# bderembl/msom

Measured on NVIDIA B200. Metric: cell-layer updates/s, higher is better.
Workload: dtype f64

## Files before the change

msom_b200/csrc/model.cu:

```cuda
#include "../../include/msqg.h"
#include "layout.cuh"
#include "mg_kernels.cuh"
#include "rb_kernels.cuh"
#include "rhs_kernels.cuh"

#include <cmath>
#include <cstdio>
#include <cstdlib>
#include <cstring>
#include <dlfcn.h>
#include <vector>
#include <utility>
#include <map>
#include <tuple>
#include <thread>
#include <mutex>
#include <condition_variable>
#include <string>
#include <atomic>

static thread_local char g_err[512] = "";
static std::mutex g_kernel_init_mu;
extern "C" const char *msqg_last_error(void) { return g_err; }
#define FAIL(code, ...)                        \
// ... 977 lines not shown
    else {
      cudaLaunchConfig_t cfg;
      memset(&cfg, 0, sizeof(cfg));
      cudaLaunchAttribute at[1];
      at[0].id = cudaLaunchAttributeClusterDimension;
      at[0].val.clusterDim.x = cs; at[0].val.clusterDim.y = 1; at[0].val.clusterDim.z = 1;
      cfg.gridDim = dim3(cs * m->num_sms); cfg.blockDim = dim3(64 * WPC); cfg.dynamicSmemBytes = smem; cfg.attrs = at; cfg.numAttrs = 1;
      int ncl = 0;
      if (cudaOccupancyMaxActiveClusters(&ncl, (void *)kern, &cfg) != cudaSuccess || ncl < 1) {
        cudaGetLastError();
        m->relax_cs_ok = false;
        if (init_lk.owns_lock()) init_lk.unlock();
        return launch_relax_ws_w<NL, K, WPC, RCOEF>(m, da, res, lev, nsweeps, C);
      }
      max_blocks[tv] = ncl * cs;
    }
    attr_set[tv].store(true, std::memory_order_release);
  }
  if (init_lk.owns_lock()) init_lk.unlock();
  const int grid = (nworkers + WPC - 1) / WPC;
  int cap = cs == 1 ? max_blocks[tv] * m->num_sms : max_blocks[tv];
  { const char *e = getenv("MSQG_RELAX_CAP"); if (e && atoi(e) > 0 && atoi(e) < cap) cap = atoi(e); }
  if (cs > 1) cap = cap < cs ? cs : cap - cap % cs;
  if (cap < 1) FAIL(MSQG_ERR_ARG, "relax kernel does not fit on the device (nl=%d)", NL);
  RelaxCoef<NL> Cc = C;
  for (int b0 = 0; b0 < grid; b0 += cap) {
    A.w_base = b0 * WPC;
    const int nb = grid - b0 < cap ? grid - b0 : cap;
    void *args[] = {(void *)&A, (void *)&Cc};
    if (cs == 1) CK(cudaLaunchCooperativeKernel((void *)kern, dim3(nb), dim3(64 * WPC), args, smem, m->stream));
    else {
      cudaLaunchConfig_t cfg;
      memset(&cfg, 0, sizeof(cfg));
      cudaLaunchAttribute at[2];
      at[0].id = cudaLaunchAttributeClusterDimension;
      at[0].val.clusterDim.x = cs; at[0].val.clusterDim.y = 1; at[0].val.clusterDim.z = 1;
      at[1].id = cudaLaunchAttributeCooperative; at[1].val.cooperative = 1;
      cfg.gridDim = dim3((nb + cs - 1) / cs * cs); cfg.blockDim = dim3(64 * WPC); cfg.dynamicSmemBytes = smem; cfg.stream = m->stream;
      cfg.attrs = at; cfg.numAttrs = 2;
      CK(cudaLaunchKernelExC(&cfg, (void *)kern, args));
    }
    m->launches++;
  }
  return MSQG_OK;
}
template <int NL>
static int launch_relax_rowcoef(msqg_model *m, double *da, const double *res, int lev, int nsweeps, const RelaxCoef<NL> &C) {
  if constexpr (NL <= 6) {
    constexpr size_t spw = WsCfg<NL, 4>::smem_per_worker;
    if constexpr (spw * 4 <= 220 * 1024) return launch_relax_ws_w<NL, 4, 4, true>(m, da, res, lev, nsweeps, C);
    else return launch_relax_ws_w<NL, 4, 2, true>(m, da, res, lev, nsweeps, C);
  } else {
    FAIL(MSQG_ERR_ARG, "varRo > 0 with the layer-coupled solver is built for nl <= 6 (nl = %d)", NL);
  }
}
template <int NL, int K>
static int launch_relax_ws(msqg_model *m, double *da, const double *res, int lev, int nsweeps, const RelaxCoef<NL> &C) {
  constexpr size_t spw = WsCfg<NL, K>::smem_per_worker;
  if constexpr (spw * 4 <= 220 * 1024) return launch_relax_ws_w<NL, K, 4>(m, da, res, lev, nsweeps, C);
  else if constexpr (spw * 2 <= 220 * 1024) return launch_relax_ws_w<NL, K, 2>(m, da, res, lev, nsweeps, C);
  else return launch_relax_ws_w<NL, K, 1>(m, da, res, lev, nsweeps, C);
}
static int relax_variant() {
#ifdef MSQG_EXPERIMENTS
  static int v = -1;
  if (v < 0) { const char *e = getenv("MSQG_RELAX"); v = (e && !strcmp(e, "v3")) ? 0 : 1; }
  return v;
#else
  return 1;
#endif
}

#ifdef MSQG_EXPERIMENTS
template <int NL, int K>
static int launch_relax_w_t(msqg_model *m, double *da, const double *res, int lev, int nsweeps, const RelaxCoef<NL> &C) {
  constexpr size_t spw = RelaxCfg<NL, K>::smem_per_warp;
  if constexpr (spw * 4 <= 200 * 1024) return launch_relax_w<NL, K, 4>(m, da, res, lev, nsweeps, C);
  else return launch_relax_w<NL, K, 2>(m, da, res, lev, nsweeps, C);
}
#endif

template <int NL>
static int launch_relax_rb(msqg_model *m, double *da, const double *res, int lev, int nrelax, const RelaxCoef<NL> &C,
                           const int *orange, int halo);
template <int NL>
static int launch_relax(msqg_model *m, double *da, const double *res, int lev, int nrelax, const RelaxCoef<NL> &C) {
  if (m->smoother == 1) return launch_relax_rb<NL>(m, da, res, lev, nrelax, C, nullptr, 0);
  int done = 0;
  while (done < nrelax) {
    int ns = nrelax - done;
    int rc;
    if (relax_uses_table<NL>(m)) { if (ns > 4) ns = 4; rc = launch_relax_rowcoef<NL>(m, da, res, lev, ns, C); }
    else if (relax_variant() == 1) { if (ns > 4) ns = 4; rc = launch_relax_ws<NL, 4>(m, da, res, lev, ns, C); }
#ifdef MSQG_EXPERIMENTS
    else if (ns <= 4) rc = launch_relax_w_t<NL, 4>(m, da, res, lev, ns, C);
    else { if (ns > 8) ns = 8; rc = launch_relax_w_t<NL, 8>(m, da, res, lev, ns, C); }
#else
    else rc = MSQG_ERR_ARG;
#endif
    if (rc) return rc;
    done += ns;
  }
  return MSQG_OK;
}


struct KernelDevState { std::atomic<bool> set[64]; int occ[64][RB_NSMAX + 1]; };
template <int NL, bool RCOEF, int WXT>
static int launch_relax_rb_pass_w(msqg_model *m, double *da, const double *res, int lev, int ns, const RelaxCoef<NL> &C,
                                const int *orange , int halo) {
  using Cfg = RbCfg<NL, WXT>;
  const Geom &g = m->g[lev];
  const int nh = 2 * ns;
  if (da != m->da.lev[lev]) FAIL(MSQG_ERR_ARG, "the rb relax pass works on the model's da list");
  if (!m->da2.lev[lev]) {
    int rc = alloc_level(m, m->da2, m->nl, lev);
    if (rc) return rc;
    m->da2.nf = m->nl;
  }
  RbArgs A;
  memset(&A, 0, sizeof(A));
  A.da = da; A.da_out = m->da2.lev[lev]; A.res = res; A.g = g; A.ns = ns;
  A.R = 2 * nh + 1 + RB_PF;
  A.TX = WXT - 2 * nh;
  A.ox_lo = 0; A.ox_hi = g.nx; A.oy_lo = 0; A.oy_hi = g.ny;
  if (orange) { A.ox_lo = orange[0]; A.ox_hi = orange[1]; A.oy_lo = orange[2]; A.oy_hi = orange[3]; }
  A.xlo = (g.bc & 1) ? -halo : 0; A.xhi = g.nx + ((g.bc & 2) ? halo : 0);
  A.ylo = (g.bc & 4) ? -halo : 0; A.yhi = g.ny + ((g.bc & 8) ? halo : 0);
  A.par0 = 0;
  A.coef = RCOEF ? relax_table(m, lev) : nullptr;
  A.coef_cell = (RCOEF && relax_table_per_cell(m)) ? 1 : 0;
  A.reuse = m->rb_reuse;
  if (RCOEF && (g.bc || !A.coef)) FAIL(MSQG_ERR_ARG, "horizontally varying stretching (varRo, frpg) is supported on undecomposed levels only");
  const int nxo_ = A.ox_hi - A.ox_lo, nyo_ = A.oy_hi - A.oy_lo;
  if constexpr (NL <= 4) {
    int lim = 512;
    { const char *e = getenv("MSQG_RB_TILE"); if (e) lim = atoi(e); }
    if (RCOEF) { const char *e = getenv("MSQG_RB_COARSE_TABLES"); if (e && atoi(e) == 0) lim = 0; }
    if ((long long)nxo_ * nyo_ <= (long long)lim * lim) {
      constexpr int WS = RB_TO + 4 * RB_NSMAX;
      const size_t tsmem = (size_t)2 * NL * WS * WS * sizeof(double);
      auto tk = k_relax_rb_tile<NL, RCOEF>;
      static KernelDevState tst;
      const int dev = m->device & 63;
      if (!tst.set[dev].load(std::memory_order_acquire)) {
        std::lock_guard<std::mutex> lk(g_kernel_init_mu);
        if (!tst.set[dev].load(std::memory_order_relaxed)) {
          CK(cudaFuncSetAttribute(tk, cudaFuncAttributeMaxDynamicSharedMemorySize, (int)tsmem));
          tst.set[dev].store(true, std::memory_order_release);
        }
      }
      RelaxCoef<NL> Cc = C;
      tk<<<dim3((nxo_ + RB_TO - 1) / RB_TO, (nyo_ + RB_TO - 1) / RB_TO), 512, tsmem, m->stream>>>(A, Cc);
      m->launches++;
      CK(cudaGetLastError());
      std::swap(m->da.lev[lev], m->da2.lev[lev]);
      if (m->swap_log) m->swap_log->push_back({m->tile_index, lev});
      return MSQG_OK;
    }
  }
  const size_t smem = (size_t)A.R * Cfg::row_bytes;
  const int threads = Cfg::NSMAX * WXT;
  auto kern = k_relax_rb<NL, RCOEF, WXT>;
  static KernelDevState st;
  const int dev = m->device & 63;
  if (!st.set[dev].load(std::memory_order_acquire)) {
    std::lock_guard<std::mutex> lk(g_kernel_init_mu);
    if (!st.set[dev].load(std::memory_order_relaxed)) {
      CK(cudaFuncSetAttribute(kern, cudaFuncAttributeMaxDynamicSharedMemorySize,
                              (int)((size_t)(4 * Cfg::NSMAX + 1 + RB_PF) * Cfg::row_bytes)));
      for (int s = 1; s <= Cfg::NSMAX; s++)
        CK(cudaOccupancyMaxActiveBlocksPerMultiprocessor(&st.occ[dev][s], kern, Cfg::NSMAX * WXT,
                                                         (size_t)(4 * s + 1 + RB_PF) * Cfg::row_bytes));
      st.set[dev].store(true, std::memory_order_release);
    }
  }
  const int occ = st.occ[dev][ns] > 0 ? st.occ[dev][ns] : 1;
  const int nxo = A.ox_hi - A.ox_lo, nyo = A.oy_hi - A.oy_lo;
  const int nstrips = (nxo + A.TX - 1) / A.TX;
  int nchunks = (m->num_sms * occ) / nstrips;
  if (nchunks > nyo / 32) nchunks = nyo / 32;
  if (nchunks < 1) nchunks = 1;
  A.rpc = (nyo + nchunks - 1) / nchunks;
  nchunks = (nyo + A.rpc - 1) / A.rpc;
  RelaxCoef<NL> Cc = C;
  kern<<<dim3(nstrips, nchunks), threads, smem, m->stream>>>(A, Cc);
  m->launches++;
  CK(cudaGetLastError());
  std::swap(m->da.lev[lev], m->da2.lev[lev]);
  if (m->swap_log) m->swap_log->push_back({m->tile_index, lev});
  return MSQG_OK;
}
template <int NL, bool RCOEF>
static int launch_relax_rb_pass(msqg_model *m, double *da, const double *res, int lev, int ns, const RelaxCoef<NL> &C,
                                const int *orange, int halo) {
#ifdef MSQG_EXPERIMENTS
  int wx = 128;
  { const char *e = getenv("MSQG_RB_WX"); if (e) wx = atoi(e); }
  if constexpr (NL <= 4) {
    const Geom &g = m->g[lev];
    const long long cells = (long long)(orange ? orange[1] - orange[0] : g.nx) * (orange ? orange[3] - orange[2] : g.ny);
    long long minside = 1024;
    { const char *e = getenv("MSQG_RB_WX_MIN"); if (e) minside = atoi(e); }
    if (wx == 64 && cells >= minside * minside) return launch_relax_rb_pass_w<NL, RCOEF, 64>(m, da, res, lev, ns, C, orange, halo);
  }
#endif
  return launch_relax_rb_pass_w<NL, RCOEF, RB_WX>(m, da, res, lev, ns, C, orange, halo);
}
template <int NL>
static int launch_relax_rb(msqg_model *m, double *da, const double *res, int lev, int nrelax, const RelaxCoef<NL> &C,
                           const int *orange = nullptr, int halo = 0) {
  constexpr int NSMAX = RbCfg<NL>::NSMAX;
  int left = nrelax;
  if (da != m->da.lev[lev]) FAIL(MSQG_ERR_ARG, "the rb relax pass works on the model's da list");
  if (orange && nrelax > NSMAX) FAIL(MSQG_ERR_ARG, "a tile relax pass holds at most %d sweeps", NSMAX);
  while (left > 0) {
    const int passes = (left + NSMAX - 1) / NSMAX;
    const int ns = (left + passes - 1) / passes;
    int rc;
    if (relax_uses_table<NL>(m)) {
      if constexpr (NL <= 6) rc = launch_relax_rb_pass<NL, true>(m, m->da.lev[lev], res, lev, ns, C, orange, halo);
      else FAIL(MSQG_ERR_ARG, "varRo > 0 with the layer-coupled solver is built for nl <= 6 (nl = %d)", NL);
    } else
      rc = launch_relax_rb_pass<NL, false>(m, m->da.lev[lev], res, lev, ns, C, orange, halo);
    if (rc) return rc;
    left -= ns;
  }
  return MSQG_OK;
}

static int coarse_top_level(msqg_model *m, int nf_problem, int maxlevel) {
  if (m->smoother != 1) return 0;
  if (nf_problem > 1 && !m->s_uniform && (m->nl > 6 || !m->rowcoef[1] || m->g[1].bc)) return 0;
  if (nf_problem == 1 && !m->modes_uniform && !m->modecoef[0][1]) return 0;
  { const char *e = getenv("MSQG_RB_COARSE_TABLES");
    if (e && atoi(e) == 0 && (nf_problem > 1 ? !m->s_uniform : !m->modes_uniform)) return 0; }
  if (!m->periodic) { const char *e = getenv("MSQG_RB_COARSE"); if (e && atoi(e) == 0) return 0; }
  int Lc = coarse_max_level(nf_problem);
  if (Lc > maxlevel) Lc = maxlevel;
  return Lc >= 2 ? Lc : 0;
}
template <int NL, bool RCOEF = false>
static int launch_coarse_rb(msqg_model *m, int Lc, int nrelax, const CoarseCoef<NL> &CC) {
  CoarseArgs A;
  memset(&A, 0, sizeof(A));
  A.res = m->res.lev[Lc]; A.da = m->da.lev[Lc]; A.g = m->g[Lc]; A.Lc = Lc; A.nrelax = nrelax; A.periodic = m->periodic;
  if (RCOEF) {
    for (int l = 1; l <= Lc; l++) {
      A.coef[l] = relax_table(m, l);
      if (!A.coef[l]) FAIL(MSQG_ERR_ARG, "no coefficient table on level %d", l);
    }
    A.coef_cell = relax_table_per_cell(m) ? 1 : 0;
  }
  size_t cells = 0;
  for (int l = 1; l <= Lc; l++) cells += (size_t)1 << (2 * l);
  const size_t smem = 2 * (size_t)NL * cells * sizeof(double);
  auto kern = k_coarse_rb<NL, RCOEF>;
  static KernelDevState st;
  const int dev = m->device & 63;
  if (!st.set[dev].load(std::memory_order_acquire)) {
    std::lock_guard<std::mutex> lk(g_kernel_init_mu);
    if (!st.set[dev].load(std::memory_order_relaxed)) {
      CK(cudaFuncSetAttribute(kern, cudaFuncAttributeMaxDynamicSharedMemorySize, RB_COARSE_SMEM));
      st.set[dev].store(true, std::memory_order_release);
    }
  }
  CoarseCoef<NL> Cc = CC;
  kern<<<1, 512, smem, m->stream>>>(A, Cc);
  m->launches++;
  CK(cudaGetLastError());
  return MSQG_OK;
}

#define NL_CASE(n, ...) case n: { constexpr int NL = n; __VA_ARGS__; } break;
#define NL_SWITCH(nl, ...)                                  \
  switch (nl) {                                             \
    NL_CASE(2, __VA_ARGS__) NL_CASE(3, __VA_ARGS__) NL_CASE(4, __VA_ARGS__) NL_CASE(5, __VA_ARGS__)   \
    NL_CASE(6, __VA_ARGS__) NL_CASE(7, __VA_ARGS__) NL_CASE(8, __VA_ARGS__) NL_CASE(9, __VA_ARGS__)   \
    NL_CASE(10, __VA_ARGS__) NL_CASE(11, __VA_ARGS__) NL_CASE(12, __VA_ARGS__)                        \
    default: FAIL(MSQG_ERR_ARG, "unsupported nl=%d", nl);   \
  }

template <class T>
__global__ void k_to_host(T *__restrict__ dst_mapped, const T *__restrict__ src, int n) {
  const int i = threadIdx.x;
  if (i < n) dst_mapped[i] = src[i];
  __threadfence_system();
}
template <class T>
static inline cudaError_t to_host(cudaStream_t st, T *host_mapped, const T *dev, int n) {
  k_to_host<T><<<1, 64, 0, st>>>(host_mapped, dev, n);
  return cudaGetLastError();
}

__global__ void k_zero_words(double *p, int n) { if ((int)threadIdx.x < n) p[threadIdx.x] = 0.; }
static inline cudaError_t zero_words(cudaStream_t st, double *p, int n) {
  k_zero_words<<<1, 64, 0, st>>>(p, n);
  return cudaGetLastError();
}

static int check_relax_err(msqg_model *m) {
  CK(to_host(m->stream, m->h_err, m->d_err, 1));
  CK(cudaStreamSynchronize(m->stream));
  if (*m->h_err) {
    CK(cudaMemsetAsync(m->d_err, 0, sizeof(int), m->stream));
    k_fill_u64<<<m->num_sms * 4, 256, 0, m->stream>>>(m->mailbox, m->mailbox_words, MAIL_EMPTY);
    FAIL(MSQG_ERR_CUDA, "relax wavefront timed out waiting on a neighbour strip");
// ... 32 lines not shown
  if (rc) return rc;
  CK(cudaStreamSynchronize(m->stream));
  *maxres = m->h_scal[0];
  return MSQG_OK;
}

template <class F>
static int run_graphed(cudaStream_t st, GraphCache &gc, const GraphKey &key, std::vector<msqg_model *> &models, long *exchanges, bool enabled,
                       F body) {
  if (!enabled) return body();
  auto it = gc.entries.find(key);
  if (it != gc.entries.end()) {
    GraphEntry &E = it->second;
    CK(cudaGraphLaunch(E.exec, st));
    for (auto &sw : E.swaps) { msqg_model *m = models[sw.first]; std::swap(m->da.lev[sw.second], m->da2.lev[sw.second]); }
    models[0]->launches += E.launches;
    if (exchanges) *exchanges += E.exchanges;
    return MSQG_OK;
  }
  if (gc.seen[key]++ == 0) return body();
  GraphEntry E;
  long l0 = 0, x0 = exchanges ? *exchanges : 0;
  for (msqg_model *m : models) { l0 += m->launches; m->swap_log = &E.swaps; }
  cudaError_t e = cudaStreamBeginCapture(st, cudaStreamCaptureModeRelaxed);
  int rc = e == cudaSuccess ? body() : MSQG_ERR_CUDA;
  cudaGraph_t g = nullptr;
  cudaError_t e2 = cudaStreamEndCapture(st, &g);
  long l1 = 0;
  for (msqg_model *m : models) { l1 += m->launches; m->swap_log = nullptr; }
  if (e != cudaSuccess || rc || e2 != cudaSuccess || !g) {
    if (g) cudaGraphDestroy(g);
    cudaGetLastError();
    if (rc) return rc;
    FAIL(MSQG_ERR_CUDA, "recording the multigrid cycle as a CUDA graph failed: %s", cudaGetErrorString(e != cudaSuccess ? e : e2));
  }
  e = cudaGraphInstantiate(&E.exec, g, 0);
  cudaGraphDestroy(g);
  if (e != cudaSuccess) FAIL(MSQG_ERR_CUDA, "cudaGraphInstantiate: %s", cudaGetErrorString(e));
  E.launches = l1 - l0; E.exchanges = exchanges ? *exchanges - x0 : 0;
  CK(cudaGraphLaunch(E.exec, st));
  gc.entries[key] = E;
  return MSQG_OK;
}
static unsigned long long da_parity_mask(msqg_model *m) {
  unsigned long long mask = 0;
  for (int l = 1; l <= m->depth; l++)
    if (m->da.lev[l] && m->da.base[l] && m->da.lev[l] != m->da.base[l] + (size_t)(m->fy[l] - 1) * m->g[l].pitch) mask |= 1ull << l;
  return mask;
}

static int mg_fused(msqg_model *m, const MgProblem &P) {
#ifdef MSQG_EXPERIMENTS
  static int v = -1;
  if (v < 0) { const char *e = getenv("MSQG_MG"); v = (e && !strcmp(e, "rr")) ? 1 : (e && !strcmp(e, "fused")) ? 2 : 0; }
  const Geom &g = m->g[m->depth];
  return (P.mode < 0 && g.bc == 0 && m->depth >= 1 && !(g.nx & 1) && !(g.ny & 1) && m->smoother == 0) ? v : 0;
#else
  (void)m; (void)P;
  return 0;
#endif
}
#ifdef MSQG_EXPERIMENTS
static int mg_corr_residual(msqg_model *m, const MgProblem &P, const double *da, double *a_new, double *maxres) {
  const int D = m->depth;
  const Geom &g = m->g[D];
  CK(zero_words(m->stream, m->d_scal, 1));
  dim3 b(CR_BX, CR_BY);
  double *res_c = (D - 1 >= 1) ? m->res.lev[D - 1] : nullptr;
  const Geom &gc = m->g[D >= 1 ? D - 1 : 0];
  { ProfScope ps(m, PROF_RESIDUAL, 0);
    LayerMetrics M = metrics_of(m);
    if (da) { NL_SWITCH(m->nl, k_corr_res<NL, true><<<grid2(g.nx, g.ny, b), b, 0, m->stream>>>(P.a, da, a_new, P.b, m->res.lev[D], res_c, m->str.lev[D], g, gc, M, m->d_scal)); }
    else { NL_SWITCH(m->nl, k_corr_res<NL, false><<<grid2(g.nx, g.ny, b), b, 0, m->stream>>>(P.a, nullptr, nullptr, P.b, m->res.lev[D], res_c, m->str.lev[D], g, gc, M, m->d_scal)); }
  }
  m->launches++;
  CK(cudaGetLastError());
  CK(to_host(m->stream, m->h_scal, m->d_scal, 1));
  CK(cudaStreamSynchronize(m->stream));
  *maxres = m->h_scal[0];
  return MSQG_OK;
}

#endif
static int mg_levels(msqg_model *m, int nf, int mode, int nrelax, int from, int top) {
  dim3 b(32, 8);
  const int D = m->depth;
  const int Lc = coarse_top_level(m, nf, top < D ? top : D - 1);
  if (m->periodic && Lc < top) FAIL(MSQG_ERR_ARG, "periodic level %d is not covered by the wrap-around coarse kernel (levels 1 .. %d)", top, Lc);
  for (int l = from - 1; l >= (Lc ? Lc : 1); l--) {
    ProfScope ps(m, PROF_RESTRICT, l);
    k_restrict<<<grid2(m->g[l].nx, m->g[l].ny, b, nf), b, 0, m->stream>>>(m->res.lev[l + 1], m->res.lev[l], m->g[l + 1], m->g[l], -1., 0);
    m->launches++;
  }
  CK(cudaGetLastError());
  int rc = MSQG_OK;
  if (Lc) {
    ProfScope ps(m, PROF_RELAX_COARSE, nrelax);
    if (mode < 0) {
      NL_SWITCH(m->nl, {
        CoarseCoef<NL> CC;
        for (int l = 1; l <= Lc; l++) CC.c[l] = relax_coef_layers<NL>(m, l);
        CC.c[0] = CC.c[1];
        if (relax_uses_table<NL>(m)) {
          if constexpr (NL <= 6) rc = launch_coarse_rb<NL, true>(m, Lc, nrelax, CC);
          else rc = MSQG_ERR_ARG;
        } else
          rc = launch_coarse_rb<NL>(m, Lc, nrelax, CC);
      });
    } else {
      CoarseCoef<1> CC;
      for (int l = 1; l <= Lc; l++) CC.c[l] = relax_coef_scalar(m, l, m->lam_lev[(size_t)l * m->nl + mode]);
      CC.c[0] = CC.c[1];
      m->coef_mode = m->modes_uniform ? -1 : mode;
      rc = m->coef_mode >= 0 ? launch_coarse_rb<1, true>(m, Lc, nrelax, CC) : launch_coarse_rb<1>(m, Lc, nrelax, CC);
      m->coef_mode = -1;
    }
    if (rc) return rc;
  }
  const int minlevel = top < 1 ? top : 1;
  for (int l = Lc ? Lc + 1 : minlevel; l <= top; l++) {
    const Geom &g = m->g[l];
    if (l == minlevel) {
      CK(cudaMemsetAsync(m->da.lev[l], 0, (size_t)nf * g.plane * sizeof(double), m->stream));
    } else {
      ProfScope ps(m, PROF_PROLONG, l);
      launch_prolong(m->stream, nf, m->da.lev[l - 1], m->da.lev[l], m->g[l - 1], g);
      m->launches++;
      CK(cudaGetLastError());
    }
    ProfScope ps(m, l == D ? PROF_RELAX_FINE : PROF_RELAX_COARSE, nrelax);
    if (mode < 0) {
      NL_SWITCH(m->nl, { auto C = relax_coef_layers<NL>(m, l); rc = launch_relax<NL>(m, m->da.lev[l], m->res.lev[l], l, nrelax, C); });
    } else {
      auto C = relax_coef_scalar(m, l, m->lam_lev[(size_t)l * m->nl + mode]);
      m->coef_mode = m->modes_uniform ? -1 : mode;
      rc = launch_relax<1>(m, m->da.lev[l], m->res.lev[l], l, nrelax, C);
      m->coef_mode = -1;
    }
    if (rc) return rc;
  }
  return MSQG_OK;
}

static int mg_cycle(msqg_model *m, const MgProblem &P, int nrelax, int fused = 0) {
  const int D = m->depth;
  dim3 b(32, 8);
  int rc = mg_levels(m, P.nf, P.mode, nrelax, fused ? D - 1 : D, D);
  if (rc) return rc;
  if (fused == 2) return MSQG_OK;
  const Geom &g = m->g[D];
  { ProfScope ps(m, PROF_CORRECT, 0);
  k_correct<<<grid2(g.nx, g.ny, b, P.nf), b, 0, m->stream>>>(P.a, m->da.lev[D], g); }
  m->launches++;
  CK(cudaGetLastError());
  return MSQG_OK;
}

static int mg_solve(msqg_model *m, const MgProblem &P, double tolerance, msqg_mgstats *st) {
  msqg_mgstats s;
  memset(&s, 0, sizeof(s));
  s.nrelax = 4;
  double resb;
  int rc;
  const int fmode = mg_fused(m, P);
#ifdef MSQG_EXPERIMENTS
  if (fmode == 1) {
    if ((rc = mg_corr_residual(m, P, nullptr, nullptr, &resb))) return rc;
    s.resb = s.resa = resb;
    for (s.i = 0; s.i < 100 && (s.i < 1 || s.resa > tolerance); s.i++) {
      if ((rc = mg_cycle(m, P, s.nrelax, 1))) return rc;
      if ((rc = mg_corr_residual(m, P, nullptr, nullptr, &s.resa))) return rc;
      if (s.resa > tolerance) {
        if (resb / s.resa < 1.2 && s.nrelax < 100) s.nrelax++;
        else if (resb / s.resa > 10 && s.nrelax > 2) s.nrelax--;
      }
      resb = s.resa;
    }
  } else if (fmode == 2) {
    const int D = m->depth;
    if (!m->a_alt.lev[D] || m->a_alt.nf < P.nf) {
      free_list(m->a_alt);
      if ((rc = alloc_list(m, m->a_alt, P.nf, -1., D, D))) return rc;
    }
    MgProblem Q = P;
    double *other = m->a_alt.lev[D];
    if ((rc = mg_corr_residual(m, Q, nullptr, nullptr, &resb))) return rc;
    s.resb = s.resa = resb;
    for (s.i = 0; s.i < 100 && (s.i < 1 || s.resa > tolerance); s.i++) {
      if ((rc = mg_cycle(m, Q, s.nrelax, 2))) return rc;
      if ((rc = mg_corr_residual(m, Q, m->da.lev[D], other, &s.resa))) return rc;
      std::swap(Q.a, other);
      if (s.resa > tolerance) {
        if (resb / s.resa < 1.2 && s.nrelax < 100) s.nrelax++;
        else if (resb / s.resa > 10 && s.nrelax > 2) s.nrelax--;
      }
      resb = s.resa;
    }
    if (Q.a != P.a) {
      if (P.owner && *P.owner == P.a) { *P.owner = Q.a; m->a_alt.lev[D] = P.a; }
      else CK(cudaMemcpyAsync(P.a, Q.a, (size_t)P.nf * m->g[D].plane * sizeof(double), cudaMemcpyDeviceToDevice, m->stream));
    }
  } else
#else
  (void)fmode;
#endif
  {
  rc = mg_residual(m, P, &resb);
  if (rc) return rc;
  s.resb = s.resa = resb;
  const bool graphed = m->smoother == 1 && m->use_graphs && !m->prof_on;
  std::vector<msqg_model *> self(1, m);
  for (s.i = 0; s.i < 100 && (s.i < 1 || s.resa > tolerance); s.i++) {
    GraphKey key(s.nrelax, P.mode, (const void *)P.a, (const void *)P.b, da_parity_mask(m));
    rc = run_graphed(m->stream, m->graphs, key, self, nullptr, graphed, [&]() -> int {
      int r2 = mg_cycle(m, P, s.nrelax);
      if (r2) return r2;
      return mg_residual_enqueue(m, P);
    });
    if (rc) return rc;
    CK(cudaStreamSynchronize(m->stream));
    s.resa = m->h_scal[0];
    if (s.resa > tolerance) {
      if (resb / s.resa < 1.2 && s.nrelax < 100) s.nrelax++;
      else if (resb / s.resa > 10 && s.nrelax > 2) s.nrelax--;
    }
    resb = s.resa;
  }
  }
  if ((rc = check_relax_err(m))) return rc;
  m->total_cycles += s.i;
  *st = s;
  return MSQG_OK;
// ... 1078 lines not shown
```

msom_b200/csrc/rb_kernels.cuh:

```cuda
#pragma once
#include "mg_kernels.cuh"

#define RB_WX 128
#define RB_NP 64
#define RB_PF 4
#define RB_NSMAX 4

struct RbArgs {
  const double *da;
  double *da_out;
  const double *res;
  Geom g;
  int ns;
  int R;
  int TX;
  int rpc;
  int ox_lo, ox_hi, oy_lo, oy_hi;
  int xlo, xhi, ylo, yhi;
  int par0;
  const double *coef;
  int coef_cell;
  int reuse;
};

__device__ __forceinline__ void cp_async8(unsigned smem_addr, const void *gsrc) {
  asm volatile("cp.async.ca.shared.global [%0], [%1], 8;\n" ::"r"(smem_addr), "l"(gsrc));
}

template <int NL, int WXT = RB_WX>
struct RbCfg {
  static constexpr int NL2 = (NL + 1) / 2;
  static constexpr int ARR2 = NL2 * WXT;
  static constexpr int ROW2 = 2 * ARR2;
  static constexpr size_t row_bytes = (size_t)ROW2 * 16;
  static constexpr int NSMAX = NL <= 4 ? RB_NSMAX : (NL <= 8 ? 2 : 1);
  static_assert((size_t)(4 * NSMAX + 1 + RB_PF) * row_bytes <= 227 * 1024, "ring does not fit");
};

template <int NL, bool RCOEF, int WXT = RB_WX>
__global__ void __launch_bounds__(RbCfg<NL, WXT>::NSMAX * WXT, WXT == 64 ? 2 : 1)
k_relax_rb(RbArgs A, RelaxCoef<NL> C) {
  using Cfg = RbCfg<NL, WXT>;
  constexpr int WX = WXT, NP = WXT / 2, PF = RB_PF, NSMAX = Cfg::NSMAX;
  constexpr int NL2 = Cfg::NL2, ARR2 = Cfg::ARR2, ROW2 = Cfg::ROW2;
  constexpr int EPT = (2 * NL + NSMAX - 1) / NSMAX;
  constexpr int EPO = (NL + NSMAX - 1) / NSMAX;
  extern __shared__ double2 ring[];
  const int tid = threadIdx.x;
  const int nh = 2 * A.ns, H = nh;
  const int k = tid / NP, p = tid % NP;
  const int pitch = A.g.pitch, nx = A.g.nx, ny = A.g.ny, bc = A.g.bc;
  const long long plane = (long long)A.g.plane;
  const int ox0 = A.ox_lo + blockIdx.x * A.TX;
  const int ox1 = min(ox0 + A.TX, A.ox_hi);
  const int x0w = ox0 - H;
  const int oy0 = A.oy_lo + blockIdx.y * A.rpc;
  const int oy1 = min(oy0 + A.rpc, A.oy_hi);
  const int jw0 = max(A.ylo, oy0 - H), jw1 = min(A.yhi, oy1 + H);
  const int nrw = jw1 - jw0;

  const int wx = tid % WX, q0 = tid / WX;
  const int gxl = x0w + wx;
  const bool lvalid = gxl >= A.xlo && gxl < A.xhi;
  const bool ovalid = gxl >= ox0 && gxl < ox1;
  const int colofs = ((wx & 1) * NP + (wx >> 1)) * 2;
  double *ring_d = reinterpret_cast<double *>(ring);
  const unsigned ring_s = (unsigned)__cvta_generic_to_shared(ring_d);
  const double *src[EPT];
  unsigned dofs[EPT];
  bool pok[EPT];
#pragma unroll
  for (int i = 0; i < EPT; i++) {
    const int q = q0 + i * NSMAX;
    pok[i] = lvalid && q < 2 * NL;
    const int arr = q >= NL ? 1 : 0, l = arr ? q - NL : q;
    src[i] = (arr ? A.res : A.da) + (pok[i] ? (long long)l * plane + (long long)(jw0 + 1) * pitch + MSQG_OX + gxl : 0);
    dofs[i] = (unsigned)((arr * 2 * ARR2 + (l >> 1) * 2 * WX + (l & 1) + colofs) * 8);
  }
  double *dst[EPO];
  unsigned sofs[EPO];
  bool sok[EPO];
#pragma unroll
  for (int i = 0; i < EPO; i++) {
    const int q = q0 + i * NSMAX;
    sok[i] = ovalid && q < NL;
    dst[i] = A.da_out + (sok[i] ? (long long)q * plane + (long long)(jw0 + 1) * pitch + MSQG_OX + gxl : 0);
    sofs[i] = (unsigned)((q >> 1) * 2 * WX + (q & 1) + colofs);
  }
  int ld_row = 0;
  unsigned ld_off = 0;
  const unsigned ROWB = (unsigned)Cfg::row_bytes, RTOTB = (unsigned)A.R * ROWB;
  auto load_row = [&]() {
    if (ld_row < nrw) {
#pragma unroll
      for (int i = 0; i < EPT; i++)
        if (pok[i]) { cp_async8(ring_s + ld_off + dofs[i], src[i]); src[i] += pitch; }
    }
    cp_async_commit();
    ld_row++;
    ld_off = ld_off + ROWB == RTOTB ? 0u : ld_off + ROWB;
  };
#pragma unroll 1
  for (int r = 0; r < PF; r++) load_row();

  int r = -1 - 2 * k;
  unsigned slB = (unsigned)(((-1 - 2 * k) % A.R + A.R) % A.R) * ROWB;
  int upd = (jw0 + r + k + A.par0 + x0w) & 1;
  unsigned cuB = (unsigned)(upd * NP + p) * 16u, ciB = (unsigned)((1 - upd) * NP + p) * 16u;
  const unsigned co0B = (unsigned)(NP + (p > 0 ? p - 1 : 0)) * 16u, co1B = (unsigned)(p < NP - 1 ? p + 1 : NP - 1) * 16u;
  const int gxa = x0w + 2 * p, gxb = gxa + 1;
  const bool exa = gxa >= A.xlo && gxa < A.xhi, exb = gxb >= A.xlo && gxb < A.xhi;
  const int pl = !(bc & 1), pr = !(bc & 2);
  const int xg0 = ((gxa == 0 && pl) ? 1 : 0) | ((gxa == nx - 1 && pr) ? 2 : 0);
  const int xg1 = ((gxb == nx - 1 && pr) ? 1 : 0) | ((gxb == 0 && pl) ? 2 : 0);
  const int r_bot = (bc & 4) ? -(1 << 30) : -jw0, r_top = (bc & 8) ? -(1 << 30) : ny - 1 - jw0;
  const bool stage_on = k < nh;
  const bool no_reuse = A.reuse == 0;
  constexpr unsigned LPB = WX * 16u;
  constexpr unsigned RESB = ARR2 * 16u;
  int ro = -2 * nh;
  unsigned soB = (unsigned)(((-2 * nh) % A.R + A.R) % A.R) * ROWB;
  const int ro_lo = oy0 - jw0, ro_hi = oy1 - jw0;
  const int T = nrw + 2 * nh;

  double F0[NL], F1[NL], F2[NL];
#pragma unroll
  for (int l = 0; l < NL; l++) { F0[l] = 0.; F1[l] = 0.; F2[l] = 0.; }

  auto step = [&](double (&Fn)[NL], double (&Fi)[NL], double (&Fs)[NL]) {
    load_row();
    if (stage_on && (unsigned)r < (unsigned)nrw) {
      const unsigned rowc = ring_s + slB;
      const unsigned rown = ring_s + (slB + ROWB == RTOTB ? 0u : slB + ROWB);
      const unsigned coB = upd ? co1B : co0B;
      double b[NL], vo[NL];
#pragma unroll
      for (int lp = 0; lp < NL2; lp++) {
        const double2 tb = lds2(rowc + RESB + lp * LPB + cuB);
        const double2 tn = lds2(rown + lp * LPB + cuB);
        const double2 to = lds2(rowc + lp * LPB + coB);
        b[2 * lp] = tb.x; Fn[2 * lp] = tn.x; vo[2 * lp] = to.x;
        if (2 * lp + 1 < NL) { b[2 * lp + 1] = tb.y; Fn[2 * lp + 1] = tn.y; vo[2 * lp + 1] = to.y; }
      }
      if (r == 0 || no_reuse) {
        const unsigned rows = ring_s + (slB == 0 ? RTOTB - ROWB : slB - ROWB);
#pragma unroll
        for (int lp = 0; lp < NL2; lp++) {
          const double2 ti = lds2(rowc + lp * LPB + ciB);
          const double2 ts = lds2(rows + lp * LPB + cuB);
          Fi[2 * lp] = ti.x; Fs[2 * lp] = ts.x;
          if (2 * lp + 1 < NL) { Fi[2 * lp + 1] = ti.y; Fs[2 * lp + 1] = ts.y; }
        }
      }
      double sh[NL], sv[NL];
      const int xg = upd ? xg1 : xg0;
      const bool gb = r == r_bot, gt = r == r_top;
      if (xg != 0 || gb || gt) {
#pragma unroll
        for (int lp = 0; lp < NL2; lp++) {
          const double2 tc = lds2(rowc + lp * LPB + cuB);
#pragma unroll
          for (int h = 0; h < 2; h++) {
            const int l = 2 * lp + h;
            if (l < NL) {
              const double g = h ? -tc.y : -tc.x;
              const double o = (xg & 1) ? g : vo[l], i = (xg & 2) ? g : Fi[l];
              const double s_ = gb ? g : Fs[l], n_ = gt ? g : Fn[l];
              sh[l] = i + o;
              sv[l] = n_ + s_;
            }
          }
        }
      } else {
#pragma unroll
        for (int l = 0; l < NL; l++) { sh[l] = Fi[l] + vo[l]; sv[l] = Fn[l] + Fs[l]; }
      }
      double rhs[NL], out[NL];
#pragma unroll
      for (int l = 0; l < NL; l++) {
        double rr = C.msd2 * b[l];
        rr += sh[l];
        rr += sv[l];
        rhs[l] = rr;
      }
      if (!RCOEF) {
#pragma unroll
        for (int l = 1; l < NL; l++) rhs[l] -= div_by(C.t0[l] * rhs[l - 1], C.t1p[l - 1], C.rinv[l - 1]);
        out[NL - 1] = div_by(rhs[NL - 1], C.t1p[NL - 1], C.rinv[NL - 1]);
#pragma unroll
        for (int l = NL - 2; l >= 0; l--) out[l] = div_by(rhs[l] - C.t2[l] * out[l + 1], C.t1p[l], C.rinv[l]);
      } else {
        const int j = jw0 + r, gx = upd ? gxb : gxa;
        const int jc = j < 0 ? 0 : (j > ny - 1 ? ny - 1 : j), xc = gx < 0 ? 0 : (gx > nx - 1 ? nx - 1 : gx);
        const double *ct = A.coef + (A.coef_cell ? (size_t)jc * nx + xc : (size_t)jc) * 6 * NL;
        double t0[NL], t2[NL], t1p[NL], rinv[NL];
#pragma unroll
        for (int l = 0; l < NL; l++) { t0[l] = ct[l]; t2[l] = ct[NL + l]; t1p[l] = ct[2 * NL + l]; rinv[l] = ct[3 * NL + l]; }
#pragma unroll
        for (int l = 1; l < NL; l++) rhs[l] -= div_by(t0[l] * rhs[l - 1], t1p[l - 1], rinv[l - 1]);
        out[NL - 1] = div_by(rhs[NL - 1], t1p[NL - 1], rinv[NL - 1]);
#pragma unroll
        for (int l = NL - 2; l >= 0; l--) out[l] = div_by(rhs[l] - t2[l] * out[l + 1], t1p[l], rinv[l]);
      }
      if (upd ? exb : exa) {
#pragma unroll
        for (int lp = 0; lp < NL2; lp++)
          sts2(rowc + lp * LPB + cuB, out[2 * lp], (2 * lp + 1 < NL) ? out[2 * lp + 1] : 0.);
      }
    }
    r++;
    slB = slB + ROWB == RTOTB ? 0u : slB + ROWB;
    upd ^= 1;
    { const unsigned tmp = cuB; cuB = ciB; ciB = tmp; }
    if (ro >= ro_lo && ro < ro_hi) {
#pragma unroll
      for (int i = 0; i < EPO; i++)
        if (sok[i]) {
          double v;
          asm volatile("ld.shared.f64 %0, [%1];" : "=d"(v) : "r"(ring_s + soB + sofs[i] * 8u));
          *dst[i] = v;
        }
    }
    if (ro >= 0) {
#pragma unroll
      for (int i = 0; i < EPO; i++) dst[i] += pitch;
    }
    ro++;
    soB = soB + ROWB == RTOTB ? 0u : soB + ROWB;
    cp_async_wait<PF - 1>();
    __syncthreads();
  };

#pragma unroll 1
  for (int t = 0; t < T; t += 3) {
    step(F0, F2, F1);
    if (t + 1 < T) step(F1, F0, F2);
    if (t + 2 < T) step(F2, F1, F0);
  }
  cp_async_wait<0>();
}

#define RB_COARSE_MAXLEV 5
template <int NL>
struct CoarseCoef { RelaxCoef<NL> c[RB_COARSE_MAXLEV + 1]; };
struct CoarseArgs {
  const double *res;
  double *da;
  Geom g;
  int Lc, nrelax;
  const double *coef[RB_COARSE_MAXLEV + 1];
  int coef_cell;
  int periodic;
};
template <int NL>
__device__ __forceinline__ size_t coarse_smem_doubles(int Lc) {
  size_t cells = 0;
  for (int l = 1; l <= Lc; l++) cells += (size_t)1 << (2 * l);
  return 2 * (size_t)NL * cells;
}
template <int NL, bool RCOEF = false>
__global__ void __launch_bounds__(512)
k_coarse_rb(CoarseArgs A, CoarseCoef<NL> CC) {
  extern __shared__ double csm[];
  const int tid = threadIdx.x, nt = blockDim.x;
  const int Lc = A.Lc;
  int base[RB_COARSE_MAXLEV + 2];
  {
    int o = 0;
    for (int l = 1; l <= Lc; l++) { base[l] = o; o += 2 * NL * (1 << (2 * l)); }
  }
  auto DA = [&](int l, int f, int y, int x) -> double & { const int n = 1 << l; return csm[base[l] + (f * n + y) * n + x]; };
  auto RS = [&](int l, int f, int y, int x) -> double & { const int n = 1 << l; return csm[base[l] + NL * n * n + (f * n + y) * n + x]; };
  {
    const int n = 1 << Lc;
    for (int e = tid; e < NL * n * n; e += nt) {
      const int f = e / (n * n), y = (e / n) % n, x = e % n;
      RS(Lc, f, y, x) = A.res[(size_t)f * A.g.plane + GIDX(A.g.pitch, y, x)];
    }
  }
  __syncthreads();
  for (int l = Lc - 1; l >= 1; l--) {
    const int n = 1 << l;
    for (int e = tid; e < NL * n * n; e += nt) {
      const int f = e / (n * n), y = (e / n) % n, x = e % n;
      double sum = 0.;
      sum += RS(l + 1, f, 2 * y, 2 * x);
      sum += RS(l + 1, f, 2 * y + 1, 2 * x);
      sum += RS(l + 1, f, 2 * y, 2 * x + 1);
      sum += RS(l + 1, f, 2 * y + 1, 2 * x + 1);
      RS(l, f, y, x) = sum / 4;
    }
    __syncthreads();
  }
  for (int l = 1; l <= Lc; l++) {
    const int n = 1 << l;
    if (l == 1) {
      for (int e = tid; e < NL * n * n; e += nt) csm[base[1] + e] = 0.;
    } else {
      const int nc = n >> 1;
      for (int e = tid; e < NL * n * n; e += nt) {
        const int f = e / (n * n), y = (e / n) % n, x = e % n;
        const int xc = x >> 1, yc = y >> 1, ix = (x & 1) ? 1 : -1, iy = (y & 1) ? 1 : -1;
        auto cat = [&](int xx, int yy) {
          double s = 1.;
          if (A.periodic) { xx = (xx + nc) & (nc - 1); yy = (yy + nc) & (nc - 1); }
          else {
            if (xx < 0) { xx = 0; s = -s; } else if (xx >= nc) { xx = nc - 1; s = -s; }
            if (yy < 0) { yy = 0; s = -s; } else if (yy >= nc) { yy = nc - 1; s = -s; }
          }
          return s * DA(l - 1, f, yy, xx);
        };
        DA(l, f, y, x) = (9. * cat(xc, yc) + 3. * (cat(xc + ix, yc) + cat(xc, yc + iy)) + cat(xc + ix, yc + iy)) / 16.;
      }
    }
    __syncthreads();
    const RelaxCoef<NL> &C = CC.c[l];
    const int half = n >> 1;
    for (int hs = 0; hs < 2 * A.nrelax; hs++) {
      const int colour = hs & 1;
      for (int e = tid; e < n * half; e += nt) {
// ... 128 lines not shown
```

Measured before the change: 3.830 billion.

## Fold multigrid correction into the final red-black relax pass on fine level

The last streaming red-black relax pass on the finest undecomposed level now adds its smoothed correction directly into the solution array a, and writes the boundary ghost cells itself. This removes the separate k_correct kernel and the extra read/write of da over the whole fine grid. To hide latency, the value of a is prefetched three rows ahead inside the streaming loop. The cost is extra global loads and boundary stores inside the relax kernel, plus another template instantiation. The fold is on by default and can be turned off with MSQG_RB_FOLD=0.

Result: faster. 3.953 billion (median of 6 runs) (+3.2%).

```diff
diff --git a/msom_b200/csrc/model.cu b/msom_b200/csrc/model.cu
--- a/msom_b200/csrc/model.cu
+++ b/msom_b200/csrc/model.cu
@@ -1083,10 +1083,12 @@
 
 template <int NL>
 static int launch_relax_rb(msqg_model *m, double *da, const double *res, int lev, int nrelax, const RelaxCoef<NL> &C,
-                           const int *orange, int halo);
+                           const int *orange, int halo, double *corr_a);
 template <int NL>
-static int launch_relax(msqg_model *m, double *da, const double *res, int lev, int nrelax, const RelaxCoef<NL> &C) {
-  if (m->smoother == 1) return launch_relax_rb<NL>(m, da, res, lev, nrelax, C, nullptr, 0);
+static int launch_relax(msqg_model *m, double *da, const double *res, int lev, int nrelax, const RelaxCoef<NL> &C,
+                        double *corr_a = nullptr) {
+  if (m->smoother == 1) return launch_relax_rb<NL>(m, da, res, lev, nrelax, C, nullptr, 0, corr_a);
+  if (corr_a) FAIL(MSQG_ERR_ARG, "the correction is folded into red-black passes only");
   int done = 0;
   while (done < nrelax) {
     int ns = nrelax - done;
@@ -1107,9 +1109,17 @@
 
 
 struct KernelDevState { std::atomic<bool> set[64]; int occ[64][RB_NSMAX + 1]; };
+static bool rb_tiled(int nf, bool rcoef, long long cells) {
+  if (nf > 4) return false;
+  int lim = 512;
+  { const char *e = getenv("MSQG_RB_TILE"); if (e) lim = atoi(e); }
+  if (rcoef) { const char *e = getenv("MSQG_RB_COARSE_TABLES"); if (e && atoi(e) == 0) lim = 0; }
+  return cells <= (long long)lim * lim;
+}
 template <int NL, bool RCOEF, int WXT>
 static int launch_relax_rb_pass_w(msqg_model *m, double *da, const double *res, int lev, int ns, const RelaxCoef<NL> &C,
-                                const int *orange , int halo) {
+                                const int *orange , int halo,
+                                double *corr_a = nullptr ) {
   using Cfg = RbCfg<NL, WXT>;
   const Geom &g = m->g[lev];
   const int nh = 2 * ns;
@@ -1134,11 +1144,15 @@
   A.reuse = m->rb_reuse;
   if (RCOEF && (g.bc || !A.coef)) FAIL(MSQG_ERR_ARG, "horizontally varying stretching (varRo, frpg) is supported on undecomposed levels only");
   const int nxo_ = A.ox_hi - A.ox_lo, nyo_ = A.oy_hi - A.oy_lo;
+  const bool fold = corr_a != nullptr;
+  if (fold) {
+    if (orange || halo || g.bc || WXT != RB_WX || rb_tiled(NL, RCOEF, (long long)nxo_ * nyo_))
+      FAIL(MSQG_ERR_ARG, "the correction is folded into streaming passes over a whole undecomposed level only");
+    if (!rb_can_fold(NL)) FAIL(MSQG_ERR_ARG, "nl = %d has no folded relax pass", NL);
+    A.a = corr_a;
+  }
   if constexpr (NL <= 4) {
-    int lim = 512;
-    { const char *e = getenv("MSQG_RB_TILE"); if (e) lim = atoi(e); }
-    if (RCOEF) { const char *e = getenv("MSQG_RB_COARSE_TABLES"); if (e && atoi(e) == 0) lim = 0; }
-    if ((long long)nxo_ * nyo_ <= (long long)lim * lim) {
+    if (rb_tiled(NL, RCOEF, (long long)nxo_ * nyo_)) {
       constexpr int WS = RB_TO + 4 * RB_NSMAX;
       const size_t tsmem = (size_t)2 * NL * WS * WS * sizeof(double);
       auto tk = k_relax_rb_tile<NL, RCOEF>;
@@ -1162,8 +1176,10 @@
   }
   const size_t smem = (size_t)A.R * Cfg::row_bytes;
   const int threads = Cfg::NSMAX * WXT;
-  auto kern = k_relax_rb<NL, RCOEF, WXT>;
-  static KernelDevState st;
+  auto kern = k_relax_rb<NL, RCOEF, WXT, false>;
+  if constexpr (rb_can_fold(NL) && WXT == RB_WX) { if (fold) kern = k_relax_rb<NL, RCOEF, WXT, true>; }
+  static KernelDevState sts[2];
+  KernelDevState &st = sts[fold ? 1 : 0];
   const int dev = m->device & 63;
   if (!st.set[dev].load(std::memory_order_acquire)) {
     std::lock_guard<std::mutex> lk(g_kernel_init_mu);
@@ -1188,13 +1204,16 @@
   kern<<<dim3(nstrips, nchunks), threads, smem, m->stream>>>(A, Cc);
   m->launches++;
   CK(cudaGetLastError());
-  std::swap(m->da.lev[lev], m->da2.lev[lev]);
-  if (m->swap_log) m->swap_log->push_back({m->tile_index, lev});
+  if (!fold) {
+    std::swap(m->da.lev[lev], m->da2.lev[lev]);
+    if (m->swap_log) m->swap_log->push_back({m->tile_index, lev});
+  }
   return MSQG_OK;
 }
 template <int NL, bool RCOEF>
 static int launch_relax_rb_pass(msqg_model *m, double *da, const double *res, int lev, int ns, const RelaxCoef<NL> &C,
-                                const int *orange, int halo) {
+                                const int *orange, int halo, double *corr_a = nullptr) {
+  if (corr_a) return launch_relax_rb_pass_w<NL, RCOEF, RB_WX>(m, da, res, lev, ns, C, orange, halo, corr_a);
 #ifdef MSQG_EXPERIMENTS
   int wx = 128;
   { const char *e = getenv("MSQG_RB_WX"); if (e) wx = atoi(e); }
@@ -1210,7 +1229,7 @@
 }
 template <int NL>
 static int launch_relax_rb(msqg_model *m, double *da, const double *res, int lev, int nrelax, const RelaxCoef<NL> &C,
-                           const int *orange = nullptr, int halo = 0) {
+                           const int *orange = nullptr, int halo = 0, double *corr_a = nullptr) {
   constexpr int NSMAX = RbCfg<NL>::NSMAX;
   int left = nrelax;
   if (da != m->da.lev[lev]) FAIL(MSQG_ERR_ARG, "the rb relax pass works on the model's da list");
@@ -1218,12 +1237,13 @@
   while (left > 0) {
     const int passes = (left + NSMAX - 1) / NSMAX;
     const int ns = (left + passes - 1) / passes;
+    double *ca = left == ns ? corr_a : nullptr;
     int rc;
     if (relax_uses_table<NL>(m)) {
-      if constexpr (NL <= 6) rc = launch_relax_rb_pass<NL, true>(m, m->da.lev[lev], res, lev, ns, C, orange, halo);
+      if constexpr (NL <= 6) rc = launch_relax_rb_pass<NL, true>(m, m->da.lev[lev], res, lev, ns, C, orange, halo, ca);
       else FAIL(MSQG_ERR_ARG, "varRo > 0 with the layer-coupled solver is built for nl <= 6 (nl = %d)", NL);
     } else
-      rc = launch_relax_rb_pass<NL, false>(m, m->da.lev[lev], res, lev, ns, C, orange, halo);
+      rc = launch_relax_rb_pass<NL, false>(m, m->da.lev[lev], res, lev, ns, C, orange, halo, ca);
     if (rc) return rc;
     left -= ns;
   }
@@ -1422,9 +1442,13 @@
 }
 
 #endif
-static int mg_levels(msqg_model *m, int nf, int mode, int nrelax, int from, int top) {
+static bool rb_fold_enabled() { const char *e = getenv("MSQG_RB_FOLD"); return !(e && atoi(e) == 0); }
+static int mg_levels(msqg_model *m, int nf, int mode, int nrelax, int from, int top, double *corr_a = nullptr,
+                     bool *corrected = nullptr) {
   dim3 b(32, 8);
   const int D = m->depth;
+  const bool fold = corrected && m->smoother == 1 && !m->periodic && rb_fold_enabled();
+  if (corrected) *corrected = false;
   const int Lc = coarse_top_level(m, nf, top < D ? top : D - 1);
   if (m->periodic && Lc < top) FAIL(MSQG_ERR_ARG, "periodic level %d is not covered by the wrap-around coarse kernel (levels 1 .. %d)", top, Lc);
   for (int l = from - 1; l >= (Lc ? Lc : 1); l--) {
@@ -1460,6 +1484,8 @@
   const int minlevel = top < 1 ? top : 1;
   for (int l = Lc ? Lc + 1 : minlevel; l <= top; l++) {
     const Geom &g = m->g[l];
+    const bool rcoef = mode < 0 ? !m->s_uniform : !m->modes_uniform;
+    double *ca = (fold && l == D && rb_can_fold(nf) && g.bc == 0 && !rb_tiled(nf, rcoef, (long long)g.nx * g.ny)) ? corr_a : nullptr;
     if (l == minlevel) {
       CK(cudaMemsetAsync(m->da.lev[l], 0, (size_t)nf * g.plane * sizeof(double), m->stream));
     } else {
@@ -1470,14 +1496,15 @@
     }
     ProfScope ps(m, l == D ? PROF_RELAX_FINE : PROF_RELAX_COARSE, nrelax);
     if (mode < 0) {
-      NL_SWITCH(m->nl, { auto C = relax_coef_layers<NL>(m, l); rc = launch_relax<NL>(m, m->da.lev[l], m->res.lev[l], l, nrelax, C); });
+      NL_SWITCH(m->nl, { auto C = relax_coef_layers<NL>(m, l); rc = launch_relax<NL>(m, m->da.lev[l], m->res.lev[l], l, nrelax, C, ca); });
     } else {
       auto C = relax_coef_scalar(m, l, m->lam_lev[(size_t)l * m->nl + mode]);
       m->coef_mode = m->modes_uniform ? -1 : mode;
-      rc = launch_relax<1>(m, m->da.lev[l], m->res.lev[l], l, nrelax, C);
+      rc = launch_relax<1>(m, m->da.lev[l], m->res.lev[l], l, nrelax, C, ca);
       m->coef_mode = -1;
     }
     if (rc) return rc;
+    if (ca) *corrected = true;
   }
   return MSQG_OK;
 }
@@ -1485,9 +1512,10 @@
 static int mg_cycle(msqg_model *m, const MgProblem &P, int nrelax, int fused = 0) {
   const int D = m->depth;
   dim3 b(32, 8);
-  int rc = mg_levels(m, P.nf, P.mode, nrelax, fused ? D - 1 : D, D);
+  bool corrected = false;
+  int rc = mg_levels(m, P.nf, P.mode, nrelax, fused ? D - 1 : D, D, fused ? nullptr : P.a, fused ? nullptr : &corrected);
   if (rc) return rc;
-  if (fused == 2) return MSQG_OK;
+  if (fused == 2 || corrected) return MSQG_OK;
   const Geom &g = m->g[D];
   { ProfScope ps(m, PROF_CORRECT, 0);
   k_correct<<<grid2(g.nx, g.ny, b, P.nf), b, 0, m->stream>>>(P.a, m->da.lev[D], g); }
diff --git a/msom_b200/csrc/rb_kernels.cuh b/msom_b200/csrc/rb_kernels.cuh
--- a/msom_b200/csrc/rb_kernels.cuh
+++ b/msom_b200/csrc/rb_kernels.cuh
@@ -21,11 +21,15 @@
   const double *coef;
   int coef_cell;
   int reuse;
+  double *a;
 };
 
 __device__ __forceinline__ void cp_async8(unsigned smem_addr, const void *gsrc) {
   asm volatile("cp.async.ca.shared.global [%0], [%1], 8;\n" ::"r"(smem_addr), "l"(gsrc));
 }
+
+__host__ __device__ constexpr int rb_nsmax(int nl) { return nl <= 4 ? RB_NSMAX : (nl <= 8 ? 2 : 1); }
+__host__ __device__ constexpr bool rb_can_fold(int nl) { return rb_nsmax(nl) > 1; }
 
 template <int NL, int WXT = RB_WX>
 struct RbCfg {
@@ -33,11 +37,11 @@
   static constexpr int ARR2 = NL2 * WXT;
   static constexpr int ROW2 = 2 * ARR2;
   static constexpr size_t row_bytes = (size_t)ROW2 * 16;
-  static constexpr int NSMAX = NL <= 4 ? RB_NSMAX : (NL <= 8 ? 2 : 1);
+  static constexpr int NSMAX = rb_nsmax(NL);
   static_assert((size_t)(4 * NSMAX + 1 + RB_PF) * row_bytes <= 227 * 1024, "ring does not fit");
 };
 
-template <int NL, bool RCOEF, int WXT = RB_WX>
+template <int NL, bool RCOEF, int WXT = RB_WX, bool FOLD = false>
 __global__ void __launch_bounds__(RbCfg<NL, WXT>::NSMAX * WXT, WXT == 64 ? 2 : 1)
 k_relax_rb(RbArgs A, RelaxCoef<NL> C) {
   using Cfg = RbCfg<NL, WXT>;
@@ -45,6 +49,7 @@
   constexpr int NL2 = Cfg::NL2, ARR2 = Cfg::ARR2, ROW2 = Cfg::ROW2;
   constexpr int EPT = (2 * NL + NSMAX - 1) / NSMAX;
   constexpr int EPO = (NL + NSMAX - 1) / NSMAX;
+  static_assert(!FOLD || rb_can_fold(NL), "no FOLD instance for this layer count");
   extern __shared__ double2 ring[];
   const int tid = threadIdx.x;
   const int nh = 2 * A.ns, H = nh;
@@ -77,6 +82,7 @@
     src[i] = (arr ? A.res : A.da) + (pok[i] ? (long long)l * plane + (long long)(jw0 + 1) * pitch + MSQG_OX + gxl : 0);
     dofs[i] = (unsigned)((arr * 2 * ARR2 + (l >> 1) * 2 * WX + (l & 1) + colofs) * 8);
   }
+  const bool corr = FOLD && A.a != nullptr;
   double *dst[EPO];
   unsigned sofs[EPO];
   bool sok[EPO];
@@ -84,7 +90,7 @@
   for (int i = 0; i < EPO; i++) {
     const int q = q0 + i * NSMAX;
     sok[i] = ovalid && q < NL;
-    dst[i] = A.da_out + (sok[i] ? (long long)q * plane + (long long)(jw0 + 1) * pitch + MSQG_OX + gxl : 0);
+    dst[i] = (corr ? A.a : A.da_out) + (sok[i] ? (long long)q * plane + (long long)(jw0 + 1) * pitch + MSQG_OX + gxl : 0);
     sofs[i] = (unsigned)((q >> 1) * 2 * WX + (q & 1) + colofs);
   }
   int ld_row = 0;
@@ -126,8 +132,11 @@
   double F0[NL], F1[NL], F2[NL];
 #pragma unroll
   for (int l = 0; l < NL; l++) { F0[l] = 0.; F1[l] = 0.; F2[l] = 0.; }
-
-  auto step = [&](double (&Fn)[NL], double (&Fi)[NL], double (&Fs)[NL]) {
+  double A0[EPO], A1[EPO], A2[EPO];
+#pragma unroll
+  for (int i = 0; i < EPO; i++) { A0[i] = 0.; A1[i] = 0.; A2[i] = 0.; }
+
+  auto step = [&](double (&Fn)[NL], double (&Fi)[NL], double (&Fs)[NL], double (&Av)[EPO]) {
     load_row();
     if (stage_on && (unsigned)r < (unsigned)nrw) {
       const unsigned rowc = ring_s + slB;
@@ -218,8 +227,30 @@
         if (sok[i]) {
           double v;
           asm volatile("ld.shared.f64 %0, [%1];" : "=d"(v) : "r"(ring_s + soB + sofs[i] * 8u));
-          *dst[i] = v;
+          if (FOLD && corr) {
+            const double w = Av[i] + v;
+            double *pa = dst[i];
+            *pa = w;
+            const int gy = jw0 + ro;
+            const bool gl = gxl == 0, gr = gxl == nx - 1, gb = gy == 0, gt = gy == ny - 1;
+            if (gl) pa[-1] = -w;
+            if (gr) pa[1] = -w;
+            if (gb) pa[-pitch] = -w;
+            if (gt) pa[pitch] = -w;
+            if (gl && gb) pa[-pitch - 1] = w;
+            if (gl && gt) pa[pitch - 1] = w;
+            if (gr && gb) pa[-pitch + 1] = w;
+            if (gr && gt) pa[pitch + 1] = w;
+          } else {
+            *dst[i] = v;
+          }
         }
+    }
+    if (FOLD && corr && ro + 3 >= ro_lo && ro + 3 < ro_hi) {
+      const int ahead = ro >= 0 ? 3 : ro + 3;
+#pragma unroll
+      for (int i = 0; i < EPO; i++)
+        if (sok[i]) Av[i] = dst[i][(long long)ahead * pitch];
     }
     if (ro >= 0) {
 #pragma unroll
@@ -233,9 +264,9 @@
 
 #pragma unroll 1
   for (int t = 0; t < T; t += 3) {
-    step(F0, F2, F1);
-    if (t + 1 < T) step(F1, F0, F2);
-    if (t + 2 < T) step(F2, F1, F0);
+    step(F0, F2, F1, A0);
+    if (t + 1 < T) step(F1, F0, F2, A1);
+    if (t + 2 < T) step(F2, F1, F0, A2);
   }
   cp_async_wait<0>();
 }
```
